# nekopanda/Amatsukaze

Measured on NVIDIA H100. Metric: 1920x1080i YV12 frames/sec (logo-eval + combing), higher is better.
Workload: dtype u8+f32

## Files before the change

### amatsukaze_b200/csrc/amtk_b200.cu

```cuda
#include "amtk_internal.h"
#include "logo_kernels.cuh"
#include "comb_kernels.cuh"
#include "comb_stream.cuh"
#include "comb_mma.cuh"
#include "scan_kernels.cuh"
#include "tnr_kernels.cuh"
#include <algorithm>
#include <cfloat>
#include <cmath>
#include <cstdlib>
#include <cstring>
#include <deque>
#include <memory>
#include <mutex>
#include <type_traits>

extern "C" { static int logo_ensure_device(const amtk_logo* cl, amtk_ctx* ctx, bool need_tables); }

namespace amtk {

static thread_local std::string g_error;
static constexpr size_t kEvalSmemLimit = 226 * 1024;
void set_error(const std::string& msg) { g_error = msg; }
bool cuda_ok(cudaError_t e, const char* what) {
// ... 299 lines not shown
}

struct CombVariant {
  int R, strip, stages, sync, TH, boxH, threads, smem;
  void (*kernel)(const CombArgs);
  void (*kernel16)(const CombArgs);
};
template <typename Cfg> static CombVariant make_variant() {
  return CombVariant{ Cfg::R, Cfg::STRIP, Cfg::STAGES, Cfg::SYNC, Cfg::TH, Cfg::BOXH, Cfg::THREADS, Cfg::SMEM, comb_tma_kernel<Cfg, 1>, nullptr };
}
template <typename Cfg> static CombVariant make_variant16() {
  return CombVariant{ Cfg::R, Cfg::STRIP, Cfg::STAGES, Cfg::SYNC, Cfg::TH, Cfg::BOXH, Cfg::THREADS, Cfg::SMEM, comb_tma_kernel<Cfg, 1>, comb_tma_kernel<Cfg, 2> };
}
static const CombVariant* comb_variants(int* n) {
  static const CombVariant v[] = {
    make_variant16<CombCfg<15, 8, 3, 0>>(), make_variant16<CombCfg<16, 8, 3, 0>>(), make_variant16<CombCfg<17, 8, 3, 0>>(),
    make_variant<CombCfg<17, 8, 2, 0>>(), make_variant<CombCfg<17, 8, 4, 0>>(), make_variant<CombCfg<17, 8, 3, 1>>(),
  };
  *n = (int)(sizeof(v) / sizeof(v[0]));
  return v;
}

static int pick_comb_R(int hY, int hC) {
  int best = 16; long long best_waste = -1;
  for (int R = 17; R >= 15; --R) {
    const int th = 8 * R;
    const long long waste = (long long)((hY + th - 1) / th) * th - hY + 2LL * (((hC + th - 1) / th) * th - hC) / 2;
    if (best_waste < 0 || waste < best_waste) { best_waste = waste; best = R; }
  }
  return best;
}

struct WsVariant { int R, stages, warps, bps, TH, boxH, smem; bool band; void (*kernel)(const WsArgs); };
template <typename Cfg> static WsVariant make_ws() { return WsVariant{ Cfg::R, Cfg::STAGES, Cfg::WARPS, Cfg::BPS, Cfg::TH, Cfg::BOXH, Cfg::SMEM, Cfg::BAND, comb_ws_kernel<Cfg> }; }
static const WsVariant* ws_variants(int* n) {
  static const WsVariant v[] = { make_ws<WsCfg<17, 2>>(), make_ws<WsCfg<15, 2>>(), make_ws<WsCfg<16, 2>>(), make_ws<WsCfg<9, 2>>(), make_ws<WsCfg<15, 3>>(), make_ws<WsCfg<12, 2>>(), make_ws<WsCfg<10, 2>>(),
                                 make_ws<WsCfg<15, 2, 7>>(), make_ws<WsCfg<13, 2, 5>>(), make_ws<WsCfg<15, 2, 2>>(), make_ws<WsCfg<15, 3, 3>>(),
                                 make_ws<WsCfg<15, 2, 4, 2>>(), make_ws<WsCfg<16, 2, 4, 2>>(), make_ws<WsCfg<17, 2, 4, 2>>(),
                                 make_ws<WbCfg<15, 2>>(), make_ws<WbCfg<16, 2>>(), make_ws<WbCfg<17, 2>>(), make_ws<WbCfg<15, 3>>(),
                                 make_ws<WtCfg<15, 2>>(), make_ws<WtCfg<16, 2>>() };
  *n = (int)(sizeof(v) / sizeof(v[0]));
  return v;
}
static int pick_ws_R(int hY, int hC, int runs = kWsRuns) {
  int best = 17; long long best_waste = -1;
  for (int R : { 17, 16, 15 }) {
    const int th = runs * R;
    const long long waste = 2LL * ((long long)((hY + th - 1) / th) * th - hY) + 2LL * ((long long)((hC + th - 1) / th) * th - hC);
    if (best_waste < 0 || waste < best_waste) { best_waste = waste; best = R; }
  }
  return best;
}

static int ws_watchdog_ok(amtk_ctx* ctx) {
  if (!ctx->watch_pending) return 1;
  AMTK_CUDA(cudaEventSynchronize(ctx->ev_watch));
  ctx->watch_pending = false;
  const int* d = ctx->ws_watch;
  if (d[0]) {
    char msg[256];
    snprintf(msg, sizeof(msg), "comb_ws (band form): a device-side wait of the previous launch timed out (wait %d, step %d, CTA %d, thread %d, parity %d); its counters are not valid",
             d[1], d[2], d[3], d[4], d[5]);
    AMTK_FAIL(msg);
  }
  return 1;
}

static const int* ws_watch_record(const amtk_ctx* ctx) {
  return ctx->plan.dev.at<const int>(ctx->plan.q_off) + 16;
}

static CUtensorMapL2promotion comb_l2_promotion(const amtk_ctx* ctx) {
  switch (ctx->knobs.comb_l2) {
    case 0: return CU_TENSOR_MAP_L2_PROMOTION_NONE;
    case 64: return CU_TENSOR_MAP_L2_PROMOTION_L2_64B;
    case 256: return CU_TENSOR_MAP_L2_PROMOTION_L2_256B;
    default: return CU_TENSOR_MAP_L2_PROMOTION_L2_128B;
  }
}

template <typename Launch>
static int comb_launch(amtk_ctx* ctx, int* counts, int nf, Launch launch) {
  AMTK_CUDA(cudaMemsetAsync(counts, 0, (size_t)nf * 12 * sizeof(int), ctx->stream));
  std::pair<EventHandle, EventHandle> ev;
  if (ctx->timing) {
    if (!ctx->timing_pool.empty()) { ev = std::move(ctx->timing_pool.back()); ctx->timing_pool.pop_back(); }
    else { AMTK_CUDA(cudaEventCreate(ev.first.put())); AMTK_CUDA(cudaEventCreate(ev.second.put())); }
    AMTK_CUDA(cudaEventRecord(ev.first, ctx->stream));
  }
  launch();
  AMTK_CUDA(cudaGetLastError());
  if (ctx->timing) { AMTK_CUDA(cudaEventRecord(ev.second, ctx->stream)); ctx->timing_events.push_back(std::move(ev)); }
  ctx->launches += 1;
  return 1;
}

static_assert(std::has_unique_object_representations<amtk_ctx::CombPlanKey>::value, "plan keys are compared with memcmp");

template <typename Build>
static int comb_plan(amtk_ctx* ctx, const amtk_ctx::CombPlanKey& key, WsArgs& args, Build build) {
  amtk_ctx::CombPlan& plan = ctx->plan;
  if (!plan.valid || memcmp(&plan.key, &key, sizeof(key)) != 0) {
    const std::vector<CombSegment> segs = build();
    const size_t seg_bytes = segs.size() * sizeof(CombSegment);
    plan.q_off = (seg_bytes + 255) & ~(size_t)255;
    plan.valid = false;
    if (!plan.dev.ensure(plan.q_off + 256)) return 0;
    AMTK_CUDA(cudaMemcpyAsync(plan.dev.at(), segs.data(), seg_bytes, cudaMemcpyHostToDevice, ctx->stream));
    AMTK_CUDA(cudaStreamSynchronize(ctx->stream));
    plan.nitems = (int)segs.size(); plan.key = key; plan.valid = true;
  }
  AMTK_CUDA(cudaMemsetAsync(plan.dev.at(plan.q_off), 0, 256, ctx->stream));
  args.segs = plan.dev.at<const CombSegment>();
  args.nitems = plan.nitems;
  args.queue = plan.dev.at<int>(plan.q_off);
  return 1;
}

static const WsVariant* ws_variant(const amtk_ctx* ctx, const amtk_clip* clip, bool tall = true) {
  const int hY = clip->height, hC = clip->height >> clip->log_uvy;
  int nvar = 0; const WsVariant* vars = ws_variants(&nvar);
  const int bps = clip->bytes_per_sample;
  const bool band = bps == 1 && ctx->knobs.comb_ws_band && ctx->knobs.comb_ws_warps == kWsWarps;
  auto find = [&](int runs, int warps) -> const WsVariant* {
    const int R = ctx->knobs.comb_R ? ctx->knobs.comb_R : pick_ws_R(hY, hC, runs);
    for (int i = 0; i < nvar; ++i)
      if (vars[i].R == R && vars[i].stages == ctx->knobs.comb_ws_stages && vars[i].warps == warps && vars[i].bps == bps && vars[i].band == band) return &vars[i];
    return nullptr;
  };
  if (band && tall && ctx->knobs.comb_ws_band == 2)
    if (const WsVariant* V = find(kWtGroups * kWsRuns, kWtGroups * kWsWarps)) return V;
  return find(kWsRuns, ctx->knobs.comb_ws_warps);
}

static int launch_comb_ws(amtk_ctx* ctx, const amtk_clip* clip, const Window& win, int lo, int hi,
                          const amtk_comb_params* prm, int* dcounts, int out_row0, const ScanItemJob* lj = nullptr) {
  const int hY = clip->height, hC = clip->height >> clip->log_uvy;
  const int wY = clip->width, wC = clip->width >> clip->log_uvx;
  const int bps = clip->bytes_per_sample;
  const WsVariant* V = ws_variant(ctx, clip);
  if (!V) AMTK_FAIL("comb: no warp-stream kernel variant for the requested AMTK_COMB_* settings");
  const bool band = V->band;
  if (lj && !band) AMTK_FAIL("comb: logo items need the band form");
  const int WW = V->warps;
  if (!ws_watchdog_ok(ctx)) return 0;
  WsArgs args;
  memset(&args, 0, sizeof(args));
  const CUtensorMapL2promotion promo = comb_l2_promotion(ctx);
  for (int pl = 0; pl < 3; ++pl) {
    const long long off = pl == 0 ? 0 : (pl == 1 ? clip->off_u : clip->off_v);
    cuuint64_t gdim[3] = { (cuuint64_t)(pl ? wC : wY) * bps, (cuuint64_t)(pl ? hC : hY), (cuuint64_t)win.count };
    cuuint64_t gstr[2] = { (cuuint64_t)(pl ? clip->pitch_uv : clip->pitch_y), (cuuint64_t)clip->frame_stride };
    cuuint32_t box[3] = { (cuuint32_t)(band ? kWbHalf : kWsTW), (cuuint32_t)V->boxH, 1u };
    if (encode_map(ctx, &args.map[pl], CU_TENSOR_MAP_DATA_TYPE_UINT8, 3, win.dev_base + off, gdim, gstr, box, CU_TENSOR_MAP_SWIZZLE_NONE, promo) != CUDA_SUCCESS)
      AMTK_FAIL("cuTensorMapEncodeTiled failed");
  }
  const int remC = (wC * bps) % kWsTW;
  const long long uv_dist = clip->off_v - clip->off_u;
  const bool pair_uv = !band && ctx->knobs.comb_merge_uv && remC > 0 && remC <= kWsTW / 2 && uv_dist > 0 && (uv_dist & 15) == 0;
  if (pair_uv) {
    cuuint64_t gdim[4] = { (cuuint64_t)wC * bps, 2u, (cuuint64_t)hC, (cuuint64_t)win.count };
    cuuint64_t gstr[3] = { (cuuint64_t)uv_dist, (cuuint64_t)clip->pitch_uv, (cuuint64_t)clip->frame_stride };
    cuuint32_t box[4] = { (cuuint32_t)(kWsTW / 2), 2u, (cuuint32_t)V->boxH, 1u };
    if (encode_map(ctx, &args.map_uv, CU_TENSOR_MAP_DATA_TYPE_UINT8, 4, win.dev_base + clip->off_u, gdim, gstr, box, CU_TENSOR_MAP_SWIZZLE_NONE, promo) != CUDA_SUCCESS)
      AMTK_FAIL("cuTensorMapEncodeTiled(uv pair) failed");
  }
  const int tyY = (hY + V->TH - 1) / V->TH, tyC = (hC + V->TH - 1) / V->TH;
  int tile0 = 0, nc = 0;
  auto thresholds = [&](WsClass& C, bool chroma) {
    C.cls = chroma ? 1 : 0; C.H = chroma ? hC : hY;
    const int tM = chroma ? prm->th_move_c : prm->th_move_y, tS = chroma ? prm->th_shima_c : prm->th_shima_y, tL = chroma ? prm->th_lshima_c : prm->th_lshima_y;
    if (bps == 1) {
      C.thM = (unsigned)(0x80 - tM) * 0x01010101u;
      C.thS = (unsigned)tS * 0x00010001u;
      C.thL = (unsigned)tL * 0x00010001u;
    } else {
      C.thM = (unsigned)std::min(tM, 2047) * 0x00010001u;
      C.thS = (unsigned)(8192 + std::min(tS, 8191)) * 0x00010001u;
      C.thL = (unsigned)(8192 + std::min(tL, 8191)) * 0x00010001u;
    }
  };
  for (int pl = 0; pl < 3; ++pl) {
    WsClass& C = args.cl[nc];
    const int w = (pl ? wC : wY) * bps;
    C.kind = 0; C.map = pl; C.W = w; thresholds(C, pl != 0);
    C.tilesX = band ? (w + kWbW - 1) / kWbW : (pl && pair_uv) ? w / kWsTW : (w + kWsTW - 1) / kWsTW;
    C.tile0 = tile0; C.ntiles = C.tilesX * (pl ? tyC : tyY);
    if (C.ntiles == 0) continue;
    tile0 += C.ntiles; ++nc;
  }
  if (pair_uv) {
    WsClass& C = args.cl[nc];
    C.kind = 1; C.x0 = wC * bps - remC; C.tilesX = 1; thresholds(C, true);
    C.tile0 = tile0; C.ntiles = tyC; tile0 += C.ntiles; ++nc;
  }
  args.nclasses = nc;
  const int ntiles = tile0, nf = hi - lo;
  amtk_ctx::CombPlan& plan = ctx->plan;
  if (plan.occ_kernel != (const void*)V->kernel) {
    int occ = 0;
    AMTK_CUDA(cudaFuncSetAttribute(V->kernel, cudaFuncAttributeMaxDynamicSharedMemorySize, V->smem));
    AMTK_CUDA(cudaOccupancyMaxActiveBlocksPerMultiprocessor(&occ, V->kernel, 32 * WW, V->smem));
    if (occ < 1) AMTK_FAIL("comb kernel does not fit on an SM");
    plan.occ = occ; plan.occ_kernel = (const void*)V->kernel;
  }
  int occ = plan.occ;
  if (ctx->knobs.comb_ctas > 0) occ = std::min(occ, ctx->knobs.comb_ctas);
  const int logoF = lj ? lj->frames : 0, nlogo = lj ? (nf + logoF - 1) / logoF : 0;
  const long long total = (long long)ntiles * nf + nlogo;
  const int per_cta = band ? 1 : WW;
  const int nwarps = ctx->sm_count * occ * per_cta;
  const int grid = (int)std::min<long long>((long long)ctx->sm_count * occ, (total + per_cta - 1) / per_cta);
  const int f0 = lo - win.first;
  const amtk_ctx::CombPlanKey key{ (const void*)V->kernel, wY, hY, wC, hC, ntiles, nf, f0, ctx->knobs.comb_item, ctx->knobs.comb_tail,
                                   occ * WW, nlogo, logoF };
  if (!comb_plan(ctx, key, args, [&] {
    int big = ctx->knobs.comb_item > 0 ? ctx->knobs.comb_item : 64, small = std::max(4, big / 4);
    while (big > 8 && (long long)ntiles * (nf / big) < 6LL * nwarps) { big /= 2; small = std::max(4, big / 4); }
    const int tail_frames = std::min(nf, std::max(small, (int)(nf * 0.15)));
    const int head_frames = nf - tail_frames;
    const int tiny = ctx->knobs.comb_tail;
    const int end_frames = (tiny > 0 && tiny < small) ? std::min(tail_frames, std::max(tiny, (int)(nf * 0.04))) : 0;
    const int mid_end = nf - end_frames;
    std::vector<CombSegment> segs;
    segs.reserve((size_t)ntiles * (head_frames / big + tail_frames / small + (tiny > 0 ? end_frames / tiny : 0) + 3) + nlogo);
    auto tier = [&](int fa, int fz, int step) {
      if (band) {
        for (int f = fa; f < fz; f += step)
          for (int t = 0; t < ntiles; ++t) segs.push_back(CombSegment{ t, f0 + f, f0 + std::min(fz, f + step) });
      } else {
        for (int t = 0; t < ntiles; ++t)
          for (int f = fa; f < fz; f += step) segs.push_back(CombSegment{ t, f0 + f, f0 + std::min(fz, f + step) });
      }
    };
    tier(0, head_frames, big);
    if (nlogo > 0) {
      const std::vector<CombSegment> head(segs);
      const long long nhead = (long long)head.size();
      segs.clear();
      int k = 0;
      for (long long i = 0; i <= nhead; ++i) {
        for (; k < nlogo && (2LL * k + 1) * nhead / (2LL * nlogo) <= i; ++k)
          segs.push_back(CombSegment{ -1, f0 + k * logoF, f0 + std::min(nf, (k + 1) * logoF) });
        if (i < nhead) segs.push_back(head[(size_t)i]);
      }
    }
    tier(head_frames, mid_end, small);
    if (tiny > 0) tier(mid_end, nf, tiny);
    return segs;
  }))
    return 0;
  args.counts = dcounts;
  args.out_frame0 = out_row0 - win.first;
  args.prefetch = ctx->knobs.comb_ws_prefetch;
  if (lj) args.logo = *lj;
  if (!comb_launch(ctx, dcounts + (size_t)(lo - out_row0) * 12, nf, [&] { V->kernel<<<grid, 32 * WW, V->smem, ctx->stream>>>(args); }))
    return 0;
  if (band) {
    if (!ctx->ws_watch) {
      AMTK_CUDA(cudaHostAlloc(ctx->ws_watch.put(), 8 * sizeof(int), cudaHostAllocDefault));
      AMTK_CUDA(cudaEventCreateWithFlags(ctx->ev_watch.put(), cudaEventDisableTiming));
    }
    AMTK_CUDA(cudaMemcpyAsync(ctx->ws_watch, ws_watch_record(ctx), 8 * sizeof(int), cudaMemcpyDeviceToHost, ctx->stream));
    AMTK_CUDA(cudaEventRecord(ctx->ev_watch, ctx->stream));
    ctx->watch_pending = true;
  }
  return 1;
}

static int launch_comb_mma(amtk_ctx* ctx, const amtk_clip* clip, const Window& win, int lo, int hi,
                           const amtk_comb_params* prm, int* dcounts, int out_row0) {
  const int hY = clip->height, hC = clip->height >> clip->log_uvy;
  const int wY = clip->width, wC = clip->width >> clip->log_uvx;
  WsArgs args;
  memset(&args, 0, sizeof(args));
  for (int pl = 0; pl < 3; ++pl) {
    const long long off = pl == 0 ? 0 : (pl == 1 ? clip->off_u : clip->off_v);
    cuuint64_t gdim[3] = { (cuuint64_t)(pl ? wC : wY), (cuuint64_t)(pl ? hC : hY), (cuuint64_t)win.count };
    cuuint64_t gstr[2] = { (cuuint64_t)(pl ? clip->pitch_uv : clip->pitch_y), (cuuint64_t)clip->frame_stride };
    cuuint32_t box[3] = { (cuuint32_t)kMmTW, (cuuint32_t)kMmBoxH, 1u };
    if (encode_map(ctx, &args.map[pl], CU_TENSOR_MAP_DATA_TYPE_UINT8, 3, win.dev_base + off, gdim, gstr, box, CU_TENSOR_MAP_SWIZZLE_128B,
                   comb_l2_promotion(ctx)) != CUDA_SUCCESS)
      AMTK_FAIL("cuTensorMapEncodeTiled failed");
  }
  const int tyY = (hY + kMmTH - 1) / kMmTH, tyC = (hC + kMmTH - 1) / kMmTH;
  int tile0 = 0, nc = 0;
  for (int pl = 0; pl < 3; ++pl) {
    WsClass& C = args.cl[nc];
    const bool chroma = pl != 0;
    C.kind = 0; C.map = pl; C.cls = chroma ? 1 : 0; C.H = chroma ? hC : hY;
    C.thM = (unsigned)(0x80 - (chroma ? prm->th_move_c : prm->th_move_y)) * 0x01010101u;
    C.thS = (unsigned)(chroma ? prm->th_shima_c : prm->th_shima_y) * 0x00010001u;
    C.thL = (unsigned)(chroma ? prm->th_lshima_c : prm->th_lshima_y) * 0x00010001u;
    C.tilesX = ((chroma ? wC : wY) + kMmTW - 1) / kMmTW;
    C.tile0 = tile0; C.ntiles = C.tilesX * (chroma ? tyC : tyY);
    if (C.ntiles == 0) continue;
    tile0 += C.ntiles; ++nc;
  }
  args.nclasses = nc;
  const int ntiles = tile0, nf = hi - lo;
  amtk_ctx::CombPlan& plan = ctx->plan;
  const int NS = ctx->knobs.comb_mma == 2 ? 2 : 1;
  void (*kern)(const WsArgs) = NS == 2 ? comb_mma_kernel<2> : comb_mma_kernel<1>;
  const int smem = NS * kMmSmemPerStream + kMmBandBytes + 1024;
  if (plan.occ_kernel != (const void*)kern) {
    AMTK_CUDA(cudaFuncSetAttribute(kern, cudaFuncAttributeMaxDynamicSharedMemorySize, smem));
    int occ_q = 0;
    AMTK_CUDA(cudaOccupancyMaxActiveBlocksPerMultiprocessor(&occ_q, kern, kMmThreads, smem));
    if (occ_q < 1) AMTK_FAIL("comb_mma: kernel does not fit on an SM");
    plan.occ = occ_q; plan.occ_kernel = (const void*)kern;
  }
  int occ = plan.occ;
  if (ctx->knobs.comb_ctas > 0) occ = std::min(occ, ctx->knobs.comb_ctas);
  const int npairs_t = (ntiles + NS - 1) / NS;
  const long long total = (long long)npairs_t * nf;
  const int nstreams = ctx->sm_count * occ;
// ... 904 lines not shown
  if (!validate_clip(clip, false)) return 0;
  if (ft->host.w != dl->host.w || fb->host.w != dl->host.w || ft->host.h != dl->host.h / 2 || fb->host.h != dl->host.h / 2)
    AMTK_FAIL("field logos do not match the deint logo");
  DevSelect ds(ctx); if (!ds.ok) return 0;
  const size_t bytes = (size_t)nframes * 33 * sizeof(float);
  float* d = out;
  if (!out_on_device) { d = host_out_buffer(ctx, bytes); if (!d) return 0; }
  if (!roi_inside(dl->host, clip, clip->pitch_y / clip->bytes_per_sample)) AMTK_FAIL("logo rectangle lies outside the frame");
  if (!for_each_roi_window(ctx, clip, frame0, nframes, dl->host.imgx, dl->host.imgy, dl->host.w, dl->host.h, false, false,
                           [&](const amtk_clip& v, const Window& w, int lo, int hi, int dx, int dy) {
        return analyze_impl(ctx, &v, dx, dy, dl, ft, fb, w, lo, hi, d, frame0); }))
    return 0;
  return finish_output(ctx, out, d, bytes, out_on_device);
}

int amtk_logo_eval_fades(amtk_ctx* ctx, const amtk_clip* clip, const amtk_logo* dl, const float* fades, int nfades,
                         int frame0, int nframes, float* out, int out_on_device) {
  if (ctx && nframes == 0) return 1;
  if (!ctx || !dl || !fades || !out) AMTK_FAIL("amtk_logo_eval_fades: bad argument");
  if (nfades < 1 || nfades > kMaxFades) AMTK_FAIL("amtk_logo_eval_fades: 1..24 fade levels");
  if (!validate_clip(clip, false)) return 0;
  DevSelect ds(ctx); if (!ds.ok) return 0;
  const size_t bytes = (size_t)nframes * nfades * sizeof(float);
  float* d = out;
  if (!out_on_device) { d = host_out_buffer(ctx, bytes); if (!d) return 0; }
  const int pitch = clip->pitch_y / clip->bytes_per_sample;
  if (!roi_inside(dl->host, clip, pitch)) AMTK_FAIL("logo rectangle lies outside the frame");
  if (!for_each_roi_window(ctx, clip, frame0, nframes, dl->host.imgx, dl->host.imgy, dl->host.w, dl->host.h, false, false,
                           [&](const amtk_clip& v, const Window& w, int lo, int hi, int dx, int dy) {
        EvalSpec sp{ dl, dl->host.imgx - dx, dl->host.imgy - dy, dl->host.w, dl->host.h, 0, 0, dl->host.w, nfades, fades, 0, 0, 1 };
        return launch_eval(ctx, &v, w, lo, hi, v.pitch_y / v.bytes_per_sample, sp, d, nfades, frame0, ctx->stream, 0); }))
    return 0;
  return finish_output(ctx, out, d, bytes, out_on_device);
}

void amtk_comb_default_params(amtk_comb_params* p) {
  if (!p) return;
  p->th_move_y = 20; p->th_shima_y = 12; p->th_lshima_y = 36;
  p->th_move_c = 24; p->th_shima_c = 16; p->th_lshima_c = 48;
}

int amtk_comb_frames(amtk_ctx* ctx, const amtk_clip* clip, const amtk_comb_params* prm, int frame0, int nframes,
                     int32_t* counts, int out_on_device) {
  if (ctx && nframes == 0) return 1;
  if (!ctx || !prm || !counts) AMTK_FAIL("amtk_comb_frames: bad argument");
  if (!validate_clip(clip, true) || !comb_thresholds_ok(prm, clip->bytes_per_sample)) return 0;
  DevSelect ds(ctx); if (!ds.ok) return 0;
  const size_t bytes = (size_t)nframes * 12 * sizeof(int32_t);
  int* d = counts;
  if (!out_on_device) { if (!ctx->dout2.ensure(bytes)) return 0; d = ctx->dout2.at<int>(); }
  if (!for_each_window(ctx, clip, frame0, nframes, true, [&](const Window& w, int lo, int hi) {
        return launch_comb(ctx, clip, w, lo, hi, prm, d, frame0); }))
    return 0;
  return finish_output(ctx, counts, d, bytes, out_on_device);
}

static int scan_item_frames(const amtk_logo* lg, const amtk_ctx* ctx, const amtk_clip* clip) {
  const WsVariant* V = ws_variant(ctx, clip, false);
  if (!V) return 0;
  const size_t ring = (size_t)V->smem - 128;
  int F = 0;
  while (F < kScanItemMaxFrames && scan_item_smem_bytes(lg->host.w, lg->host.h, lg->countPad, F + 1) <= ring) ++F;
  return F;
}

int amtk_scan_comb_frames(amtk_ctx* ctx, const amtk_clip* clip, amtk_logo* const* logos, int nlogos,
                          const amtk_comb_params* prm, int frame0, int nframes, float* scores, int32_t* counts, int out_on_device) {
  if (ctx && nframes == 0) return 1;
  if (!ctx || !prm || !counts || !scores || !logos || nlogos < 1) AMTK_FAIL("amtk_scan_comb_frames: bad argument");
  if (!validate_clip(clip, true) || !comb_thresholds_ok(prm, clip->bytes_per_sample)) return 0;
  DevSelect ds(ctx); if (!ds.ok) return 0;
  const size_t sbytes = (size_t)nframes * nlogos * 2 * sizeof(float), cbytes = (size_t)nframes * 12 * sizeof(int32_t);
  float* ds_ = scores; int* dc = counts;
  if (!out_on_device) {
    if (!ctx->dout.ensure(sbytes) || !ctx->dout2.ensure(cbytes)) return 0;
    ds_ = ctx->dout.at<float>(); dc = ctx->dout2.at<int>();
  }
  const amtk_logo* lg0 = logos[0];
  const bool one_logo = nlogos == 1 && lg0 && lg0->has_mask && lg0->host.count() > 0 &&
                        lg0->host.imgw == clip->width && lg0->host.imgh == clip->height && lg0->host.imgx >= 0 && lg0->host.imgy >= 0 &&
                        lg0->host.imgx + lg0->host.w <= clip->width && lg0->host.imgy + lg0->host.h <= clip->height;
  if (!for_each_window(ctx, clip, frame0, nframes, true, [&](const Window& w, int lo, int hi) -> int {
        const WsVariant* V = one_logo && comb_runs_band(ctx, clip, w) ? ws_variant(ctx, clip) : nullptr;
        const int F = V ? scan_item_frames(lg0, ctx, clip) : 0;
        if (F > 0) {
          if (!logo_ensure_device(lg0, ctx, true)) return 0;
          ScanItemJob lj;
          lj.ybase = w.dev_base; lj.frame_stride = clip->frame_stride; lj.pitch = clip->pitch_y;
          lj.imgx = lg0->host.imgx; lj.imgy = lg0->host.imgy;
          lj.logo = logo_dev(lg0); lj.maxv = (float)((1 << clip->bits_per_sample) - 1);
          lj.frames = F; lj.scores = ds_;
          return launch_comb_ws(ctx, clip, w, lo, hi, prm, dc, frame0, &lj);
        }
        return launch_comb(ctx, clip, w, lo, hi, prm, dc, frame0) &&
               scan_frames_impl(ctx, clip, clip, 0, 0, logos, nlogos, w, lo, hi, 0, ds_, frame0); }))
    return 0;
  if (out_on_device) return 1;
  AMTK_CUDA(cudaMemcpyAsync(scores, ds_, sbytes, cudaMemcpyDeviceToHost, ctx->stream));
  AMTK_CUDA(cudaMemcpyAsync(counts, dc, cbytes, cudaMemcpyDeviceToHost, ctx->stream));
  AMTK_CUDA(cudaStreamSynchronize(ctx->stream));
  return 1;
}

static int scan_sample_bits(const amtk_clip* c) {
  if (c->bytes_per_sample == 1) {
    if (c->bits_per_sample <= 8) return 8;
  } else if (c->bits_per_sample > 8 && c->bits_per_sample <= 16) {
    if (((c->pitch_y | c->pitch_uv | c->off_u | c->off_v | c->frame_stride | (int64_t)reinterpret_cast<uintptr_t>(c->base)) & 1) == 0)
      return c->bits_per_sample;
    set_error("LogoScan: 2-byte clips need even pitches, plane offsets, frame stride and base");
    return 0;
  }
  set_error("LogoScan: bits_per_sample must be at most 8 for 1-byte samples and 9..16 for 2-byte samples");
  return 0;
}

int amtk_scan_create(amtk_ctx* ctx, int scanw, int scanh, int lx, int ly, int thy, amtk_scan** out) {
  if (!ctx || !out) AMTK_FAIL("amtk_scan_create: null argument");
  if (scanw < 4 || scanh < 4 || scanw > 4096 || scanh > 4096 || lx < 0 || lx > 2 || ly < 0 || ly > 2) AMTK_FAIL("amtk_scan_create: bad geometry");
  DevSelect ds(ctx); if (!ds.ok) return 0;
  std::unique_ptr<amtk_scan> s(new amtk_scan());
  s->ctx = ctx; s->device = ctx->device; s->scanw = scanw; s->scanh = scanh; s->logUVx = lx; s->logUVy = ly; s->thy = thy;
  s->npix = (size_t)scanw * scanh + 2 * (size_t)(scanw >> lx) * (scanh >> ly);
  if (!cuda_ok(cudaMalloc(s->dSums.put(), s->npix * 3 * sizeof(unsigned long long)), "cudaMalloc") ||
      !cuda_ok(cudaMalloc(s->dBg.put(), 8 * sizeof(unsigned long long)), "cudaMalloc") ||
      !cuda_ok(cudaMemsetAsync(s->dSums, 0, s->npix * 3 * sizeof(unsigned long long), ctx->stream), "cudaMemsetAsync") ||
      !cuda_ok(cudaMemsetAsync(s->dBg, 0, 8 * sizeof(unsigned long long), ctx->stream), "cudaMemsetAsync"))
    return 0;
  *out = s.release();
  return 1;
}

void amtk_scan_destroy(amtk_scan* s) {
  if (!s) return;
  DevSelect ds(s->device);
  delete s;
}

int amtk_scan_add_frames(amtk_scan* s, const amtk_clip* clip, int scanx, int scany, int frame0, int nframes,
                         const uint8_t* frame_select, uint8_t* valid_out) {
  if (!s) AMTK_FAIL("amtk_scan_add_frames: null scan");
  amtk_ctx* ctx = s->ctx;
  if (!validate_clip(clip, true)) return 0;
  const int bits = scan_sample_bits(clip);
  if (!bits) return 0;
  if (s->bytes_per_sample && (clip->bytes_per_sample != s->bytes_per_sample || bits != s->bits))
    AMTK_FAIL("LogoScan: the clip's sample format differs from the first clip's");
  if (clip->log_uvx != s->logUVx || clip->log_uvy != s->logUVy) AMTK_FAIL("chroma subsampling mismatch");
  if (scanx < 0 || scany < 0 || scanx + s->scanw > clip->width || scany + s->scanh > clip->height) AMTK_FAIL("scan rectangle outside the frame");
  if (frame0 < 0 || nframes < 0 || frame0 + nframes > clip->num_frames) AMTK_FAIL("frame range outside the clip");
  DevSelect ds(ctx); if (!ds.ok) return 0;
  s->bytes_per_sample = clip->bytes_per_sample; s->bits = bits;
  const bool wide = clip->bytes_per_sample == 2;
  const size_t bg_bytes = (size_t)nframes * sizeof(int4), off_sel = (bg_bytes + 255) & ~(size_t)255;
// ... 1153 lines not shown
```

### amatsukaze_b200/csrc/amtk_internal.h

```cpp
#pragma once
#include <cuda.h>
#include <cuda_runtime.h>
#include <algorithm>
#include <cstdint>
#include <cstdio>
#include <mutex>
#include <string>
#include <vector>
#include "../../include/amtk_b200.h"
#include "logo_host.h"

typedef CUresult (*amtk_encode_tiled_fn)(CUtensorMap*, CUtensorMapDataType, cuuint32_t, void*, const cuuint64_t*,
                                         const cuuint64_t*, const cuuint32_t*, const cuuint32_t*, CUtensorMapInterleave,
                                         CUtensorMapSwizzle, CUtensorMapL2promotion, CUtensorMapFloatOOBfill);

namespace amtk {

void set_error(const std::string& msg);
bool cuda_ok(cudaError_t e, const char* what);

#define AMTK_CUDA(call)                                          \
  do {                                                           \
    if (!::amtk::cuda_ok((call), #call)) return 0;               \
  } while (0)
// ... 51 lines not shown

struct amtk_ctx {
  mutable std::recursive_mutex mu;
  int device = 0;
  cudaStream_t stream = nullptr;
  amtk::StreamHandle owned_stream;
  amtk::StreamHandle copy_stream;
  amtk::StreamHandle side_stream, side_stream2;
  amtk::EventHandle ev_fork, ev_join1, ev_join2;
  amtk::EventHandle ev_copy[2];
  amtk::EventHandle ev_done[2];
  int sm_count = 0;
  int64_t launches = 0;
  long long h2d_bytes_last = 0;
  amtk::GrowBuf scratch;
  amtk::GrowBuf stage[2];
  amtk::GrowBuf small;
  amtk::GrowBuf dout;
  amtk::GrowBuf dout2;
  amtk::PinnedBuf<void> hout; void* hout_dev = nullptr;
  amtk_encode_tiled_fn encode_tiled = nullptr;
  struct Knobs {
    int eval_waves = 1;
    int eval_cw = 1;
    int eval_par = 1;
    int comb_generic = 0;
    int comb_merge_uv = 1;
    int comb_part = -1;
    int comb_strip = 8, comb_stages = 3, comb_R = 0, comb_ctas = 0, comb_sync = 0, comb_l2 = 64;
    int comb_item = 0;
    int comb_tail = 4;
    int comb_ws_stages = 2;
    int comb_mma = 0;
    int comb_ws10 = 0;
    int comb_ws_warps = 4;
    int comb_ws_prefetch = 0;
    int comb_ws_band = 2;
    int comb_ws = 1;
  } knobs;
  struct CombPlanKey {
    const void* kernel;
    int wY, hY, wC, hC, ntiles, nf, f0;
    int item, tail;
    int ctas;
    int nlogo, logoF;
  };
  struct CombPlan {
    bool valid = false;
    CombPlanKey key{};
    amtk::GrowBuf dev;
    int nitems = 0; size_t q_off = 0;
    int occ = 0; const void* occ_kernel = nullptr;
  } plan;
  amtk::PinnedBuf<int> ws_watch;
  amtk::EventHandle ev_watch;
  bool watch_pending = false;
  bool timing = false;
  std::vector<std::pair<amtk::EventHandle, amtk::EventHandle>> timing_events;
  std::vector<std::pair<amtk::EventHandle, amtk::EventHandle>> timing_pool;
  double timing_ms = 0.0; int64_t timing_count = 0;
};

struct amtk_logo {
  int device = -1;
  amtk::HostLogo host;
  amtk::DevBuf<float> dA, dB;
  amtk::DevBuf<float> dAU, dBU, dAV, dBV;
  amtk::DevBuf<uint32_t> dPix; amtk::DevBuf<float> dTapsT; amtk::DevBuf<float2> dScales;
  int countPad = 0;
  bool has_mask = false;
  bool tables_uploaded = false;
  std::mutex mu;
};

struct amtk_scan {
  amtk_ctx* ctx = nullptr;
  int device = 0;
  int scanw = 0, scanh = 0, logUVx = 1, logUVy = 1, thy = 0;
  int nvalid = 0;
  int bytes_per_sample = 0, bits = 0;
  amtk::DevBuf<unsigned long long> dSums;
  amtk::DevBuf<unsigned long long> dBg;
  size_t npix = 0;
};
```

### amatsukaze_b200/csrc/comb_stream.cuh

```cuda
#pragma once
#include <cuda_fp16.h>
#include "amtk_internal.h"
#include "tma_utils.cuh"
#include "comb_kernels.cuh"
#include "logo_kernels.cuh"

namespace amtk {

constexpr int kWsTW = 128;
constexpr int kWsRuns = 4;
constexpr int kWsWarps = 4;

template <int R_, int STAGES_, int WARPS_ = kWsWarps, int BPS_ = 1>
struct WsCfg {
  static constexpr int R = R_, STAGES = STAGES_, WARPS = WARPS_;
  static constexpr int BPS = BPS_;
  static constexpr int TH = kWsRuns * R;
  static constexpr int BOXH = TH + 4;
  static constexpr int STAGE_BYTES = kWsTW * BOXH;
  static constexpr int RING_BYTES = STAGES * STAGE_BYTES;
  static constexpr int SMEM = WARPS * RING_BYTES + 128;
  static constexpr int FIT = (227 * 1024) / (SMEM + 1024 + 8 * WARPS * STAGES + 8);
  static constexpr int MIN_CTAS = FIT >= 4 ? 4 : FIT >= 3 ? 3 : FIT >= 2 ? 2 : 1;
  static constexpr bool BAND = false;
};

constexpr int kWbW = 512;
constexpr int kWbHalf = 256;
template <int R_, int STAGES_, int GROUPS_>
struct BandCfg {
  static constexpr int R = R_, STAGES = STAGES_, GROUPS = GROUPS_, WARPS = GROUPS * (kWbW / kWsTW), BPS = 1;
  static constexpr int TH = GROUPS * kWsRuns * R;
  static constexpr int BOXH = TH + 4;
  static_assert(BOXH <= 256, "a TMA box is at most 256 rows");
  static constexpr int HALF_BYTES = kWbHalf * BOXH;
  static constexpr int STAGE_BYTES = 2 * HALF_BYTES;
  static constexpr int SMEM = STAGES * STAGE_BYTES + 128;
  static constexpr int FIT = (227 * 1024) / (SMEM + 1024 + 12 * STAGES + 16);
  static constexpr int MIN_CTAS = FIT >= 4 ? 4 : FIT >= 3 ? 3 : FIT >= 2 ? 2 : 1;
  static constexpr bool BAND = true;
};
template <int R_, int STAGES_> using WbCfg = BandCfg<R_, STAGES_, 1>;
constexpr int kWtGroups = 3;
template <int R_, int STAGES_> using WtCfg = BandCfg<R_, STAGES_, kWtGroups>;

struct WsClass {
  int tile0, ntiles;
  int kind;
  int tilesX;
  int map;
  int x0;
  int W;
  int H;
  int cls;
  unsigned thM, thS, thL;
};
constexpr int kWsMaxClasses = 4;
struct WsArgs {
  CUtensorMap map[3];
  CUtensorMap map_uv;
  WsClass cl[kWsMaxClasses];
  int nclasses;
  const CombSegment* segs;
  int nitems;
  int* queue;
  int* counts;
  int out_frame0;
  int prefetch;
  ScanItemJob logo;
};

__device__ __forceinline__ void tma_load_4d(void* smem_dst, const CUtensorMap* map, uint64_t* bar, int c0, int c1, int c2, int c3) {
  asm volatile(
      "cp.async.bulk.tensor.4d.shared::cluster.global.mbarrier::complete_tx::bytes [%0], [%1, {%3, %4, %5, %6}], [%2];"
      ::"r"(smem_u32(smem_dst)), "l"(map), "r"(smem_u32(bar)), "r"(c0), "r"(c1), "r"(c2), "r"(c3)
      : "memory");
}

__device__ __forceinline__ void tma_prefetch_3d(const CUtensorMap* map, int c0, int c1, int c2) {
  asm volatile("cp.async.bulk.prefetch.tensor.3d.L2.global.tile [%0, {%1, %2, %3}];" ::"l"(map), "r"(c0), "r"(c1), "r"(c2) : "memory");
}
__device__ __forceinline__ void tma_prefetch_4d(const CUtensorMap* map, int c0, int c1, int c2, int c3) {
  asm volatile("cp.async.bulk.prefetch.tensor.4d.L2.global.tile [%0, {%1, %2, %3, %4}];" ::"l"(map), "r"(c0), "r"(c1), "r"(c2), "r"(c3) : "memory");
}

#ifndef AMTK_WS_RELOAD_PREV
#define AMTK_WS_RELOAD_PREV 1
#endif
constexpr bool kWsReloadPrev = AMTK_WS_RELOAD_PREV != 0;
#ifndef AMTK_WS_L_VIA_IDP
#define AMTK_WS_L_VIA_IDP 0
#endif
constexpr bool kWsLviaIdp = AMTK_WS_L_VIA_IDP != 0;
__device__ __forceinline__ uint4 lds128(const uint8_t* p) {
  uint4 v;
  asm("ld.shared.v4.u32 {%0, %1, %2, %3}, [%4];" : "=r"(v.x), "=r"(v.y), "=r"(v.z), "=r"(v.w) : "r"(smem_u32(p)));
  return v;
}

struct H8 { __half2 v[8]; };

__device__ __forceinline__ H8 bytes16_to_half(const uint4 raw) {
  H8 r;
  const uint32_t w[4] = { raw.x, raw.y, raw.z, raw.w };
#pragma unroll
  for (int i = 0; i < 4; ++i) {
    uint32_t a = __byte_perm(w[i], 0, 0x4140), b = __byte_perm(w[i], 0, 0x4342);
    r.v[2 * i] = *reinterpret_cast<__half2*>(&a); r.v[2 * i + 1] = *reinterpret_cast<__half2*>(&b);
  }
  return r;
}

struct WsCounts { uint32_t S[2], L[2], M[2]; };

__device__ __forceinline__ void ws_row_masks(const H8& h0, const H8& h1, const H8& h2, const H8& h3, const H8& h4,
                                             const __half2 thS, const __half2 thL, uint32_t& accS, uint32_t& accL) {
  const __half2 k4 = __float2half2_rn(4.0f), km3 = __float2half2_rn(-3.0f);
  uint32_t mS[8], mL[8];
#pragma unroll
  for (int q = 0; q < 8; ++q) {
    __half2 t = __hadd2(h0.v[q], h4.v[q]);
    t = __hfma2(k4, h2.v[q], t);
// ... 242 lines not shown
    }
    uint32_t fix_mine = 0u;
    if (y_first < 2) fix_mine |= (1u << (2 - y_first)) - 1u;
    {
      const int lo_j = max(C.H - 2 - y_first, 0), hi_j = min(C.H + 2 - y_first, R);
      if (hi_j > lo_j) fix_mine |= ((1u << hi_j) - 1u) & ~((1u << lo_j) - 1u);
    }
    const uint32_t fix_rows = __reduce_or_sync(0xFFFFFFFFu, fix_mine);
    const int flip = y_first & 1;
    const uint32_t kM = C.thM, tS = C.thS, tL = C.thL;
    int* const crow = a.counts + C.cls * 6 + lane + ((long long)seg.fbegin - 1 - a.out_frame0) * 12;

    int st = (int)(gload % S);
    uint32_t ph = (gload / S) & 1u;
    mbar_wait(&full_bar[st], ph);
    uint4 P[R];
    {
      const uint8_t* l0 = tiles + st * Cfg::STAGE_BYTES + lane_off;
#pragma unroll
      for (int j = 0; j < R; ++j) P[j] = *reinterpret_cast<const uint4*>(l0 + (j + 2) * kWsTW);
      __syncwarp();
      if (lane == 0 && S < nloads) issue_at(S, st);
      if (lane == 0 && pf > 0 && S + pf < nloads) prefetch_at(S + pf);
    }
    for (int k = 1; k <= nf; ++k) {
      if (++st == S) { st = 0; ph ^= 1u; }
      mbar_wait(&full_bar[st], ph);
      const uint8_t* cur = tiles + st * Cfg::STAGE_BYTES + lane_off;
      WsCounts c = Cfg::BPS == 2 ? ws_rows10<R, kWsTW>(cur, P, kM, tS, tL)
                                 : (AMTK_WS_SP ? ws_rows_sp<R, kWsTW>(cur, P, kM, tS, tL) : ws_rows<R, kWsTW>(cur, P, kM, tS, tL));
      if (fix_rows) {
        if (Cfg::BPS == 2) ws_fixup10<kWsTW>(cur, fix_rows, fix_mine, tS, tL, c); else ws_fixup<kWsTW>(cur, fix_rows, fix_mine, tS, tL, c);
        __syncwarp();
      }
      const uint32_t s0 = flip ? c.S[1] : c.S[0], s1 = flip ? c.S[0] : c.S[1];
      const uint32_t l0 = flip ? c.L[1] : c.L[0], l1 = flip ? c.L[0] : c.L[1];
      const uint32_t m0 = flip ? c.M[1] : c.M[0], m1 = flip ? c.M[0] : c.M[1];
      const uint32_t rM0 = __reduce_add_sync(0xFFFFFFFFu, m0), rS0 = __reduce_add_sync(0xFFFFFFFFu, s0), rL0 = __reduce_add_sync(0xFFFFFFFFu, l0);
      const uint32_t rM1 = __reduce_add_sync(0xFFFFFFFFu, m1), rS1 = __reduce_add_sync(0xFFFFFFFFu, s1), rL1 = __reduce_add_sync(0xFFFFFFFFu, l1);
      __syncwarp();
      if (lane == 0 && (k + S) < nloads) issue_at(k + S, st);
      if (lane == 0 && pf > 0 && (k + S + pf) < nloads) prefetch_at(k + S + pf);
      if (lane < 6) {
        const int fld = lane >= 3, met = lane - 3 * fld;
        uint32_t v = met == 0 ? (fld ? rM1 : rM0) : met == 1 ? (fld ? rS1 : rS0) : (fld ? rL1 : rL0);
        v = (met == 0 && Cfg::BPS == 1) ? (v >> 7) : (met == 2 && kWsLviaIdp && Cfg::BPS == 1) ? v / 510u : decode_pair(v);
        if (v) atomicAdd(crow + (size_t)k * 12, (int)v);
      }
    }
    gload += (uint32_t)nloads;
  }
}

template <typename Cfg>
__device__ __forceinline__ void ws_bands(const WsArgs& a) {
  constexpr int S = Cfg::STAGES, R = Cfg::R, NW = Cfg::WARPS;
  extern __shared__ uint8_t smem_raw[];
  __shared__ __align__(8) uint64_t full_bar[S];
  __shared__ uint32_t released[S];
  __shared__ int item_s[2];
  const int tid = threadIdx.x, lane = tid & 31, warp = tid >> 5;
  uint8_t* slots = smem_raw + ((128u - (smem_u32(smem_raw) & 127u)) & 127u);
  if (tid == 0) {
#pragma unroll
    for (int s = 0; s < S; ++s) { mbar_init(&full_bar[s], 1); released[s] = 0u; }
    asm volatile("fence.mbarrier_init.release.cluster;" ::: "memory");
  }
  __syncthreads();
  int* const dbg = a.queue + 16;
  uint32_t gload = 0;
  const int strip = lane & 7, run = lane >> 3;
  const int col = (warp % 4) * kWsTW;
  const int grow = (warp / 4) * kWsRuns * R;
  const int lane_off = (col / kWbHalf) * Cfg::HALF_BYTES + (grow + run * R) * kWbHalf + (col % kWbHalf) + strip * 16;
  for (int it = 0;; it ^= 1) {
    if (tid == 0) item_s[it] = atomicAdd(a.queue, 1);
    __syncthreads();
    const int item = item_s[it];
    if (item >= a.nitems) break;
    const CombSegment seg = a.segs[item];
    if (seg.tile < 0) {
      scan_item<32 * NW>(a.logo, seg.fbegin, seg.fend, a.out_frame0, slots);
      asm volatile("fence.proxy.async.shared::cta;" ::: "memory");
      continue;
    }
    int ci = 0;
#pragma unroll
    for (int k = 1; k < kWsMaxClasses; ++k) if (k < a.nclasses && seg.tile >= a.cl[k].tile0) ci = k;
    const WsClass& C = a.cl[ci];
    const int lt = seg.tile - C.tile0;
    const int ty = lt / C.tilesX, tx = lt - ty * C.tilesX;
    const int y0 = ty * Cfg::TH, x0 = tx * kWbW;
    const int y_first = y0 + grow + run * R;
    const bool two = x0 + kWbHalf < C.W;
    const bool active = x0 + col < C.W && y0 + grow < C.H + 2;
    const int nf = seg.fend - seg.fbegin;
    const int nloads = nf + 1;
    const int fprev = seg.fbegin > 0 ? seg.fbegin - 1 : seg.fbegin;
    const CUtensorMap* map = &a.map[C.map];

    auto issue_at = [&](int j, int st) {
      const int fr = (j == 0) ? fprev : seg.fbegin + j - 1;
      uint8_t* dst = slots + st * Cfg::STAGE_BYTES;
      mbar_expect_tx(&full_bar[st], two ? 2 * Cfg::HALF_BYTES : Cfg::HALF_BYTES);
      tma_load_3d(dst, map, &full_bar[st], x0, y0 - 2, fr);
      if (two) tma_load_3d(dst + Cfg::HALF_BYTES, map, &full_bar[st], x0 + kWbHalf, y0 - 2, fr);
    };
    auto release = [&](int j, int st) {
      __syncwarp();
      if (lane == 0 && atomicAdd(&released[st], 1u) % NW == NW - 1 && j + S < nloads) issue_at(j + S, st);
    };
    if (tid == 0) {
      const int pro = nloads < S ? nloads : S;
      for (int j = 0; j < pro; ++j) issue_at(j, (int)((gload + (uint32_t)j) % S));
    }
    uint32_t fix_mine = 0u;
    if (y_first < 2) fix_mine |= (1u << (2 - y_first)) - 1u;
    {
      const int lo_j = max(C.H - 2 - y_first, 0), hi_j = min(C.H + 2 - y_first, R);
      if (hi_j > lo_j) fix_mine |= ((1u << hi_j) - 1u) & ~((1u << lo_j) - 1u);
    }
    const uint32_t fix_rows = __reduce_or_sync(0xFFFFFFFFu, fix_mine);
    const int flip = y_first & 1;
    const uint32_t kM = C.thM, tS = C.thS, tL = C.thL;
    int* const crow = a.counts + C.cls * 6 + lane + ((long long)seg.fbegin - 1 - a.out_frame0) * 12;

    int st = (int)(gload % S);
    uint32_t ph = (gload / S) & 1u;
    mm_wait(&full_bar[st], ph, dbg, 1, 0);
    uint4 P[R];
    if (active) {
      const uint8_t* l0 = slots + st * Cfg::STAGE_BYTES + lane_off;
#pragma unroll
      for (int j = 0; j < R; ++j) P[j] = *reinterpret_cast<const uint4*>(l0 + (j + 2) * kWbHalf);
    }
    release(0, st);
    for (int k = 1; k <= nf; ++k) {
      if (++st == S) { st = 0; ph ^= 1u; }
      mm_wait(&full_bar[st], ph, dbg, 2, k);
      if (!active) { release(k, st); continue; }
      const uint8_t* cur = slots + st * Cfg::STAGE_BYTES + lane_off;
      WsCounts c = ws_rows<R, kWbHalf>(cur, P, kM, tS, tL);
      if (fix_rows) {
        ws_fixup<kWbHalf>(cur, fix_rows, fix_mine, tS, tL, c);
        __syncwarp();
      }
      const uint32_t s0 = flip ? c.S[1] : c.S[0], s1 = flip ? c.S[0] : c.S[1];
      const uint32_t l0 = flip ? c.L[1] : c.L[0], l1 = flip ? c.L[0] : c.L[1];
      const uint32_t m0 = flip ? c.M[1] : c.M[0], m1 = flip ? c.M[0] : c.M[1];
      const uint32_t rM0 = __reduce_add_sync(0xFFFFFFFFu, m0), rS0 = __reduce_add_sync(0xFFFFFFFFu, s0), rL0 = __reduce_add_sync(0xFFFFFFFFu, l0);
      const uint32_t rM1 = __reduce_add_sync(0xFFFFFFFFu, m1), rS1 = __reduce_add_sync(0xFFFFFFFFu, s1), rL1 = __reduce_add_sync(0xFFFFFFFFu, l1);
      release(k, st);
      if (lane < 6) {
        const int fld = lane >= 3, met = lane - 3 * fld;
        uint32_t v = met == 0 ? (fld ? rM1 : rM0) : met == 1 ? (fld ? rS1 : rS0) : (fld ? rL1 : rL0);
        v = met == 0 ? (v >> 7) : (met == 2 && kWsLviaIdp) ? v / 510u : decode_pair(v);
        if (v) atomicAdd(crow + (size_t)k * 12, (int)v);
      }
    }
    gload += (uint32_t)nloads;
  }
}

template <typename Cfg>
__global__ void __launch_bounds__(32 * Cfg::WARPS, Cfg::MIN_CTAS) comb_ws_kernel(const __grid_constant__ WsArgs a) {
  if constexpr (Cfg::BAND) ws_bands<Cfg>(a); else ws_warp_streams<Cfg>(a);
}
}
```

Baseline: 882,400.

## Prefetch next band item across item boundaries and drop per-launch host watchdog work

```diff
diff --git a/amatsukaze_b200/csrc/amtk_b200.cu b/amatsukaze_b200/csrc/amtk_b200.cu
--- a/amatsukaze_b200/csrc/amtk_b200.cu
+++ b/amatsukaze_b200/csrc/amtk_b200.cu
@@ -375,22 +375,30 @@
   return best;
 }
 
-static int ws_watchdog_ok(amtk_ctx* ctx) {
+static int ws_watchdog_ok(amtk_ctx* ctx, bool wait) {
   if (!ctx->watch_pending) return 1;
-  AMTK_CUDA(cudaEventSynchronize(ctx->ev_watch));
+  if (wait) {
+    AMTK_CUDA(cudaEventSynchronize(ctx->ev_watch));
+  } else {
+    const cudaError_t e = cudaEventQuery(ctx->ev_watch);
+    if (e == cudaErrorNotReady) return 1;
+    AMTK_CUDA(e);
+  }
   ctx->watch_pending = false;
-  const int* d = ctx->ws_watch;
+  int* d = ctx->ws_watch;
   if (d[0]) {
     char msg[256];
-    snprintf(msg, sizeof(msg), "comb_ws (band form): a device-side wait of the previous launch timed out (wait %d, step %d, CTA %d, thread %d, parity %d); its counters are not valid",
+    snprintf(msg, sizeof(msg), "comb_ws (band form): a device-side wait of an earlier launch timed out (wait %d, step %d, CTA %d, thread %d, parity %d); its counters are not valid",
              d[1], d[2], d[3], d[4], d[5]);
+    memset(d, 0, 8 * sizeof(int));
+    AMTK_CUDA(cudaMemsetAsync(ctx->ws_watch_dev, 0, 8 * sizeof(int), ctx->stream));
     AMTK_FAIL(msg);
   }
   return 1;
 }
 
 static const int* ws_watch_record(const amtk_ctx* ctx) {
-  return ctx->plan.dev.at<const int>(ctx->plan.q_off) + 16;
+  return ctx->ws_watch_dev;
 }
 
 static CUtensorMapL2promotion comb_l2_promotion(const amtk_ctx* ctx) {
@@ -421,9 +429,11 @@
 static_assert(std::has_unique_object_representations<amtk_ctx::CombPlanKey>::value, "plan keys are compared with memcmp");
 
 template <typename Build>
-static int comb_plan(amtk_ctx* ctx, const amtk_ctx::CombPlanKey& key, WsArgs& args, Build build) {
+static int comb_plan(amtk_ctx* ctx, const amtk_ctx::CombPlanKey& key, WsArgs& args, Build build, bool kernel_rearms = false) {
   amtk_ctx::CombPlan& plan = ctx->plan;
+  bool reset = !kernel_rearms;
   if (!plan.valid || memcmp(&plan.key, &key, sizeof(key)) != 0) {
+    reset = true;
     const std::vector<CombSegment> segs = build();
     const size_t seg_bytes = segs.size() * sizeof(CombSegment);
     plan.q_off = (seg_bytes + 255) & ~(size_t)255;
@@ -433,7 +443,7 @@
     AMTK_CUDA(cudaStreamSynchronize(ctx->stream));
     plan.nitems = (int)segs.size(); plan.key = key; plan.valid = true;
   }
-  AMTK_CUDA(cudaMemsetAsync(plan.dev.at(plan.q_off), 0, 256, ctx->stream));
+  if (reset) AMTK_CUDA(cudaMemsetAsync(plan.dev.at(plan.q_off), 0, 256, ctx->stream));
   args.segs = plan.dev.at<const CombSegment>();
   args.nitems = plan.nitems;
   args.queue = plan.dev.at<int>(plan.q_off);
@@ -466,7 +476,17 @@
   const bool band = V->band;
   if (lj && !band) AMTK_FAIL("comb: logo items need the band form");
   const int WW = V->warps;
-  if (!ws_watchdog_ok(ctx)) return 0;
+  if (band) {
+    if (!ws_watchdog_ok(ctx, false)) return 0;
+    if (!ctx->ws_watch_dev) {
+      AMTK_CUDA(cudaHostAlloc(ctx->ws_watch.put(), 8 * sizeof(int), cudaHostAllocMapped));
+      memset(ctx->ws_watch.get(), 0, 8 * sizeof(int));
+      AMTK_CUDA(cudaHostGetDevicePointer((void**)&ctx->ws_watch_mapped, ctx->ws_watch.get(), 0));
+      AMTK_CUDA(cudaEventCreateWithFlags(ctx->ev_watch.put(), cudaEventDisableTiming));
+      AMTK_CUDA(cudaMalloc(ctx->ws_watch_dev.put(), 8 * sizeof(int)));
+      AMTK_CUDA(cudaMemsetAsync(ctx->ws_watch_dev, 0, 8 * sizeof(int), ctx->stream));
+    }
+  }
   WsArgs args;
   memset(&args, 0, sizeof(args));
   const CUtensorMapL2promotion promo = comb_l2_promotion(ctx);
@@ -571,20 +591,17 @@
     tier(head_frames, mid_end, small);
     if (tiny > 0) tier(mid_end, nf, tiny);
     return segs;
-  }))
+  }, band))
     return 0;
   args.counts = dcounts;
   args.out_frame0 = out_row0 - win.first;
   args.prefetch = ctx->knobs.comb_ws_prefetch;
   if (lj) args.logo = *lj;
+  args.watch = ctx->ws_watch_dev;
+  args.watch_host = ctx->ws_watch_mapped;
   if (!comb_launch(ctx, dcounts + (size_t)(lo - out_row0) * 12, nf, [&] { V->kernel<<<grid, 32 * WW, V->smem, ctx->stream>>>(args); }))
     return 0;
   if (band) {
-    if (!ctx->ws_watch) {
-      AMTK_CUDA(cudaHostAlloc(ctx->ws_watch.put(), 8 * sizeof(int), cudaHostAllocDefault));
-      AMTK_CUDA(cudaEventCreateWithFlags(ctx->ev_watch.put(), cudaEventDisableTiming));
-    }
-    AMTK_CUDA(cudaMemcpyAsync(ctx->ws_watch, ws_watch_record(ctx), 8 * sizeof(int), cudaMemcpyDeviceToHost, ctx->stream));
     AMTK_CUDA(cudaEventRecord(ctx->ev_watch, ctx->stream));
     ctx->watch_pending = true;
   }
@@ -1595,7 +1612,8 @@
   if (!for_each_window(ctx, clip, frame0, nframes, true, [&](const Window& w, int lo, int hi) {
         return launch_comb(ctx, clip, w, lo, hi, prm, d, frame0); }))
     return 0;
-  return finish_output(ctx, counts, d, bytes, out_on_device);
+  if (!finish_output(ctx, counts, d, bytes, out_on_device)) return 0;
+  return out_on_device ? 1 : ws_watchdog_ok(ctx, true);
 }
 
 static int scan_item_frames(const amtk_logo* lg, const amtk_ctx* ctx, const amtk_clip* clip) {
@@ -1642,7 +1660,7 @@
   AMTK_CUDA(cudaMemcpyAsync(scores, ds_, sbytes, cudaMemcpyDeviceToHost, ctx->stream));
   AMTK_CUDA(cudaMemcpyAsync(counts, dc, cbytes, cudaMemcpyDeviceToHost, ctx->stream));
   AMTK_CUDA(cudaStreamSynchronize(ctx->stream));
-  return 1;
+  return ws_watchdog_ok(ctx, true);
 }
 
 static int scan_sample_bits(const amtk_clip* c) {
diff --git a/amatsukaze_b200/csrc/amtk_internal.h b/amatsukaze_b200/csrc/amtk_internal.h
--- a/amatsukaze_b200/csrc/amtk_internal.h
+++ b/amatsukaze_b200/csrc/amtk_internal.h
@@ -127,7 +127,9 @@
     int nitems = 0; size_t q_off = 0;
     int occ = 0; const void* occ_kernel = nullptr;
   } plan;
+  amtk::DevBuf<int> ws_watch_dev;
   amtk::PinnedBuf<int> ws_watch;
+  int* ws_watch_mapped = nullptr;
   amtk::EventHandle ev_watch;
   bool watch_pending = false;
   bool timing = false;
diff --git a/amatsukaze_b200/csrc/comb_stream.cuh b/amatsukaze_b200/csrc/comb_stream.cuh
--- a/amatsukaze_b200/csrc/comb_stream.cuh
+++ b/amatsukaze_b200/csrc/comb_stream.cuh
@@ -68,6 +68,8 @@
   int out_frame0;
   int prefetch;
   ScanItemJob logo;
+  int* watch;
+  int* watch_host;
 };
 
 __device__ __forceinline__ void tma_load_4d(void* smem_dst, const CUtensorMap* map, uint64_t* bar, int c0, int c1, int c2, int c3) {
@@ -416,67 +418,108 @@
   }
 }
 
+enum : int { kWbEnd = 0, kWbStream = 1, kWbLogo = 2 };
+struct WbItem {
+  int kind;
+  int fbegin, fend;
+  int cl;
+  int map, x0, y0, two;
+};
+constexpr int kWbLogoScratch = 2 * BandCfg<17, 2, 1>::STAGE_BYTES;
+
 template <typename Cfg>
 __device__ __forceinline__ void ws_bands(const WsArgs& a) {
   constexpr int S = Cfg::STAGES, R = Cfg::R, NW = Cfg::WARPS;
+  constexpr bool kLogoInSlot = S == 2 && Cfg::STAGE_BYTES >= kWbLogoScratch;
+  static_assert(Cfg::GROUPS == 1 || kLogoInSlot, "a tall slot holds any logo item the 512 x 4R ring holds");
   extern __shared__ uint8_t smem_raw[];
   __shared__ __align__(8) uint64_t full_bar[S];
   __shared__ uint32_t released[S];
-  __shared__ int item_s[2];
+  __shared__ WbItem desc[2];
   const int tid = threadIdx.x, lane = tid & 31, warp = tid >> 5;
   uint8_t* slots = smem_raw + ((128u - (smem_u32(smem_raw) & 127u)) & 127u);
+  auto claim = [&](WbItem& D, bool more) {
+    const int item = more ? atomicAdd(a.queue, 1) : a.nitems;
+    if (item >= a.nitems) { D.kind = kWbEnd; return; }
+    const CombSegment seg = a.segs[item];
+    D.fbegin = seg.fbegin; D.fend = seg.fend;
+    if (seg.tile < 0) { D.kind = kWbLogo; return; }
+    int ci = 0;
+#pragma unroll
+    for (int k = 1; k < kWsMaxClasses; ++k) if (k < a.nclasses && seg.tile >= a.cl[k].tile0) ci = k;
+    const WsClass& C = a.cl[ci];
+    const int lt = seg.tile - C.tile0;
+    const int ty = lt / C.tilesX, tx = lt - ty * C.tilesX;
+    D.kind = kWbStream; D.cl = ci; D.map = C.map; D.x0 = tx * kWbW; D.y0 = ty * Cfg::TH; D.two = D.x0 + kWbHalf < C.W;
+  };
+  auto issue = [&](const WbItem& D, int j, int st) {
+    const int fr = j > 0 ? D.fbegin + j - 1 : (D.fbegin > 0 ? D.fbegin - 1 : D.fbegin);
+    uint8_t* dst = slots + st * Cfg::STAGE_BYTES;
+    const CUtensorMap* map = &a.map[D.map];
+    mbar_expect_tx(&full_bar[st], D.two ? 2 * Cfg::HALF_BYTES : Cfg::HALF_BYTES);
+    tma_load_3d(dst, map, &full_bar[st], D.x0, D.y0 - 2, fr);
+    if (D.two) tma_load_3d(dst + Cfg::HALF_BYTES, map, &full_bar[st], D.x0 + kWbHalf, D.y0 - 2, fr);
+  };
   if (tid == 0) {
 #pragma unroll
     for (int s = 0; s < S; ++s) { mbar_init(&full_bar[s], 1); released[s] = 0u; }
     asm volatile("fence.mbarrier_init.release.cluster;" ::: "memory");
+    claim(desc[0], true);
   }
   __syncthreads();
-  int* const dbg = a.queue + 16;
+  int* const dbg = a.watch;
   uint32_t gload = 0;
+  int c_lo = 0, c_hi = 0;
   const int strip = lane & 7, run = lane >> 3;
   const int col = (warp % 4) * kWsTW;
   const int grow = (warp / 4) * kWsRuns * R;
   const int lane_off = (col / kWbHalf) * Cfg::HALF_BYTES + (grow + run * R) * kWbHalf + (col % kWbHalf) + strip * 16;
-  for (int it = 0;; it ^= 1) {
-    if (tid == 0) item_s[it] = atomicAdd(a.queue, 1);
-    __syncthreads();
-    const int item = item_s[it];
-    if (item >= a.nitems) break;
-    const CombSegment seg = a.segs[item];
-    if (seg.tile < 0) {
-      scan_item<32 * NW>(a.logo, seg.fbegin, seg.fend, a.out_frame0, slots);
+  for (int i = 0;; i ^= 1) {
+    const WbItem* const D = &desc[i];
+    WbItem* const N = &desc[i ^ 1];
+    const int kind = D->kind;
+    if (kind == kWbEnd) break;
+    if (kind == kWbLogo) {
+      uint8_t* scratch = slots;
+      if constexpr (kLogoInSlot) scratch = slots + ((gload + 1u) % S) * Cfg::STAGE_BYTES;
+      scan_item<32 * NW>(a.logo, D->fbegin, D->fend, a.out_frame0, scratch);
+      if (tid == 0) {
+        claim(*N, true);
+        c_lo = c_hi = 0;
+        if (kLogoInSlot && N->kind == kWbStream) { issue(*N, 0, (int)(gload % S)); c_hi = 1; }
+      }
       asm volatile("fence.proxy.async.shared::cta;" ::: "memory");
+      __syncthreads();
       continue;
     }
-    int ci = 0;
-#pragma unroll
-    for (int k = 1; k < kWsMaxClasses; ++k) if (k < a.nclasses && seg.tile >= a.cl[k].tile0) ci = k;
-    const WsClass& C = a.cl[ci];
-    const int lt = seg.tile - C.tile0;
-    const int ty = lt / C.tilesX, tx = lt - ty * C.tilesX;
-    const int y0 = ty * Cfg::TH, x0 = tx * kWbW;
+    const WsClass& C = a.cl[D->cl];
+    const int y0 = D->y0, fbegin = D->fbegin;
     const int y_first = y0 + grow + run * R;
-    const bool two = x0 + kWbHalf < C.W;
-    const bool active = x0 + col < C.W && y0 + grow < C.H + 2;
-    const int nf = seg.fend - seg.fbegin;
+    const bool active = D->x0 + col < C.W && y0 + grow < C.H + 2;
+    const int nf = D->fend - fbegin;
     const int nloads = nf + 1;
-    const int fprev = seg.fbegin > 0 ? seg.fbegin - 1 : seg.fbegin;
-    const CUtensorMap* map = &a.map[C.map];
-
-    auto issue_at = [&](int j, int st) {
-      const int fr = (j == 0) ? fprev : seg.fbegin + j - 1;
-      uint8_t* dst = slots + st * Cfg::STAGE_BYTES;
-      mbar_expect_tx(&full_bar[st], two ? 2 * Cfg::HALF_BYTES : Cfg::HALF_BYTES);
-      tma_load_3d(dst, map, &full_bar[st], x0, y0 - 2, fr);
-      if (two) tma_load_3d(dst + Cfg::HALF_BYTES, map, &full_bar[st], x0 + kWbHalf, y0 - 2, fr);
-    };
+    const int jc = nloads - S > 0 ? nloads - S : 0;
+
     auto release = [&](int j, int st) {
       __syncwarp();
-      if (lane == 0 && atomicAdd(&released[st], 1u) % NW == NW - 1 && j + S < nloads) issue_at(j + S, st);
+      if (lane == 0) {
+        if (j >= jc) __threadfence_block();
+        if (atomicAdd(&released[st], 1u) % NW == NW - 1) {
+          const int jn = j + S;
+          if (jn < nloads) {
+            issue(*D, jn, st);
+          } else {
+            __threadfence_block();
+            if (N->kind == kWbStream && jn - nloads <= N->fend - N->fbegin) issue(*N, jn - nloads, st);
+          }
+        }
+      }
     };
     if (tid == 0) {
       const int pro = nloads < S ? nloads : S;
-      for (int j = 0; j < pro; ++j) issue_at(j, (int)((gload + (uint32_t)j) % S));
+      for (int j = 0; j < pro; ++j)
+        if (j < c_lo || j >= c_hi) issue(*D, j, (int)((gload + (uint32_t)j) % S));
+      if (jc == 0) claim(*N, true);
     }
     uint32_t fix_mine = 0u;
     if (y_first < 2) fix_mine |= (1u << (2 - y_first)) - 1u;
@@ -487,7 +530,7 @@
     const uint32_t fix_rows = __reduce_or_sync(0xFFFFFFFFu, fix_mine);
     const int flip = y_first & 1;
     const uint32_t kM = C.thM, tS = C.thS, tL = C.thL;
-    int* const crow = a.counts + C.cls * 6 + lane + ((long long)seg.fbegin - 1 - a.out_frame0) * 12;
+    int* const crow = a.counts + C.cls * 6 + lane + ((long long)fbegin - 1 - a.out_frame0) * 12;
 
     int st = (int)(gload % S);
     uint32_t ph = (gload / S) & 1u;
@@ -502,6 +545,7 @@
     for (int k = 1; k <= nf; ++k) {
       if (++st == S) { st = 0; ph ^= 1u; }
       mm_wait(&full_bar[st], ph, dbg, 2, k);
+      if (k == jc && tid == 0) claim(*N, true);
       if (!active) { release(k, st); continue; }
       const uint8_t* cur = slots + st * Cfg::STAGE_BYTES + lane_off;
       WsCounts c = ws_rows<R, kWbHalf>(cur, P, kM, tS, tL);
@@ -522,7 +566,21 @@
         if (v) atomicAdd(crow + (size_t)k * 12, (int)v);
       }
     }
+    if (tid == 0) {
+      c_lo = S > nloads ? S - nloads : 0;
+      c_hi = N->kind == kWbStream ? S : c_lo;
+    }
     gload += (uint32_t)nloads;
+    __syncthreads();
+  }
+  if (tid == 0) {
+    const volatile int* w = dbg;
+    if (w[0]) {
+      for (int q = 0; q < 8; ++q) a.watch_host[q] = w[q];
+      __threadfence_system();
+    }
+    __threadfence();
+    if (atomicAdd(a.queue + 1, 1) == (int)gridDim.x - 1) { a.queue[0] = 0; a.queue[1] = 0; }
   }
 }
 
```

New measurement: 900,700 (median of 6 runs). 1.02x the previous value.
